# akashsengupta1997/HierarchicalProbabilistic3DHuman

Hardware: AMD Instinct MI355X
Metric: images/sec end-to-end (num_samples=100) (higher is better)
Workload: dtype f32

## Files before the change

hierarchicalprobabilistic3dhuman_amd/_capi.py:

```python
import contextlib
import ctypes
import os

import torch

_PKG_DIR = os.path.dirname(os.path.abspath(__file__))
LIB_PATH = os.path.join(_PKG_DIR, "libhps.so")
DEV_LIB_PATH = os.path.join(_PKG_DIR, "libhps_dev.so")

_c = ctypes
_P = _c.c_void_p
_I = _c.c_int

_PROTOTYPES = {
    "hps_version": [],
    "hps_last_error": [],
    "hps_stream_create_cu_partition": [_I, _I, _c.POINTER(_P)],
    "hps_stream_destroy": [_P],
    "hps_smpl_pose_prep": [_P, _P, _I, _P, _I, _P, _P, _P, _P, _I, _P, _I, _I, _P, _P, _P, _I, _P],
    "hps_smpl_blend": [_P, _P, _P, _P, _I, _I, _I, _I, _I, _I, _P],
    "hps_smpl_lbs": [_P, _I, _P, _P, _P, _I, _I, _P, _P, _I, _I, _P],
    "hps_smpl_mesh_fused": [_P, _P, _P, _P, _P, _P, _I, _I, _P, _P, _I, _I, _I, _I, _I, _P],
    "hps_smpl_mesh_fused_picks": [_P, _P, _P, _P, _P, _P, _I, _I, _P, _P, _I, _I, _I, _I, _I, _P, _P, _I, _P],
    "hps_smpl_mesh_fused_shared_shape": [_P] * 8 + [_I, _I, _P] + [_I] * 5 + [_P, _P, _I, _P],
# ... 6 lines not shown
    "hps_smpl_lbs_backward": [_P, _I, _P, _P, _P, _I, _I, _P, _P, _I, _P, _P, _P, _P, _P, _P, _I, _I, _P],
    "hps_smpl_blend_backward": [_P, _P, _P, _P, _I, _I, _I, _I, _I, _P],
    "hps_smpl_pose_prep_backward": [_P, _P, _I, _P, _I, _P, _P, _P, _P, _I, _P, _P, _I, _P, _I, _P, _P, _P, _I, _P],
    "hps_smpl_joints": [_P, _P, _P, _P, _P, _I, _I, _P, _P, _I, _I, _P],
    "hps_vertex_uncertainty": [_P, _P, _I, _I, _I, _P],
    "hps_joints_and_uncertainty": [_P, _P, _P, _P, _P, _I, _I, _P, _P, _I, _I, _P, _P, _I, _I, _I, _P],
    "hps_query_workspace": [_I, _c.c_int64, _c.c_int64, _c.c_int64],
    "hps_mf_sample": [_P, _P, _P, _P, _P, _I, _I, _I, _I, _c.c_float, _c.c_float, _P, _P, _P, _c.c_uint64,
                      _c.c_int64, _P, _I, _P, _P, _P, _P],
    "hps_infer_assemble": [_P, _P, _P, _P, _P, _P, _P, _I, _I, _I, _I, _P],
    "hps_quat_to_rotmat": [_P, _P, _I, _P],
    "hps_rot6d_to_rotmat": [_P, _P, _I, _P],
    "hps_batch_rodrigues": [_P, _P, _I, _P],
    "hps_linear": [_P, _I, _P, _P, _P, _P, _I, _I, _I, _I, _I, _P],
    "hps_head_trunk": [_P] + [_I] + [_P] * 14 + [_I] * 7 + [_P],
    "hps_head_joint_level": [_P, _I, _I, _P, _I, _P, _P, _P, _P, _P, _P, _P, _P, _P, _c.c_float, _P, _P, _I, _I, _P],
    "hps_head_joint_level_svd": [_P, _I, _I, _P, _I, _P, _P, _P, _P, _P, _P, _P, _P, _P, _c.c_float, _P, _P, _P, _P, _I, _I, _I, _P],
    "hps_svd3_packed": [_P, _P, _I, _I, _P],
    "hps_host_svd3_emulated": [_P, _P, _I, _I],
    "hps_host_svd_flavor": [],
    "hps_host_svd3_packed": [_P, _P, _I, _I],
    "hps_host_bind_lapack": [_c.c_char_p],
    "hps_head_svd_finish": [_P, _P, _I, _P, _P, _P, _P, _P, _P, _I, _I, _P],
    "hps_canny_edges": [_P, _P, _I, _P, _P, _P, _P, _P, _P, _I, _I, _I, _I, _c.c_float, _I, _P],
    "hps_canny_edge_map": [_P, _P, _I, _P, _c.c_int64, _I, _I, _I, _I, _c.c_float, _I, _P],
    "hps_proxy_rep": [_P, _P, _P, _P, _I, _I, _I, _I, _c.c_float, _P],
    "hps_pointset_errors": [_P, _P, _I, _I, _I, _I, _P, _P, _P, _P, _P],
    "hps_heatmaps_to_joints2d": [_P, _P, _P, _I, _I, _I, _c.c_float, _P],
    "hps_sample_joints2d_error": [_P, _P, _I, _P, _P, _P, _c.c_float, _P, _I, _I, _P],
    "hps_conv2d_bn_act_pad": [_P, _P, _P, _P, _P, _P, _I, _I, _I, _I, _I, _I, _I, _I, _I, _I, _I, _I, _I, _I, _I, _P, _P],
    "hps_conv2d_bn_act_pad_down": [_P] * 9 + [_I] * 14 + [_P, _P],
    "hps_conv3x3_winograd": [_P, _P, _P, _P, _P, _P, _I, _I, _I, _I, _I, _I, _I, _I, _P, _P],
    "hps_conv3x3_winograd_workspace": [_I, _I, _I, _I, _I],
    "hps_stem_phase_frames_bytes": [_I, _I, _I],
    "hps_stem_phase_split": [_P, _P, _I, _I, _I, _I, _P],
    "hps_proxy_rep_phase_frames": [_P, _P, _P, _P, _I, _I, _I, _I, _c.c_float, _P],
    "hps_stem_winograd": [_P, _P, _P, _P, _P, _I, _I, _I, _I, _I, _P],
    "hps_stem_pool_side_bytes": [_I, _I, _I],
    "hps_stem_winograd_pooled": [_P, _P, _P, _P, _P, _P, _I, _I, _I, _I, _I, _P],
    "hps_stem_winograd_pooled_nchw": [_P, _P, _P, _P, _P, _P, _I, _I, _I, _I, _I, _P],
    "hps_sums_f64": [_P, _P, _P, _I, _c.c_double, _P, _P, _P, _P],
    "hps_sizeof_enc_op": [],
    "hps_encoder_run": [_P, _I, _P],
    "hps_head_pose_levels": [_P, _I, _I, _P, _P, _I, _P, _P, _P, _P, _P, _P, _P, _P, _P, _c.c_float, _P, _P, _P, _P, _P, _P,
                             _P, _P, _I, _I, _I, _I, _P],
    "hps_nchw_to_padded_nhwc": [_P, _P, _I, _I, _I, _I, _I, _P],
    "hps_nchw_to_padded_nhwc_generic": [_P, _P, _I, _I, _I, _I, _I, _I, _I, _P],
    "hps_maxpool3x3s2_pad": [_P, _P, _I, _I, _I, _I, _I, _P],
    "hps_global_avgpool_pad": [_P, _P, _I, _I, _I, _I, _I, _P],
    "hps_mf_log_norm_const": [_P, _I, _P, _P, _P, _P],
    "hps_mf_nll": [_P, _P, _P, _P, _P, _I, _c.c_double, _P, _P, _P, _P, _P],
    "hps_mf_loss_forward": [_P, _P, _P, _P],
    "hps_mf_loss_backward": [_P, _P, _P, _P],
    "hps_head_forward_refine": [_P, _I] + [_P] * 9 + [_I] + [_P] * 6 + [_c.c_float] + [_P] * 13 + [_I] * 7 + [_P],
    "hps_head_pose_levels_backward": [_P, _I, _I, _P, _P, _I] + [_P] * 21 + [_I, _I, _I, _P],
    "hps_head_pose_levels_backward_factors": [_P, _I, _I, _P, _P, _I] + [_P] * 23 + [_I, _I, _I, _P],
    "hps_mf_sample_keep_quat": [_P, _P, _P, _I, _I, _I, _I, _c.c_float, _c.c_float, _P, _P, _P, _c.c_uint64, _c.c_int64, _I, _P, _P, _P, _P],
    "hps_mf_sample_backward": [_P, _P, _P, _P, _P, _P, _P, _P, _I, _I, _I, _c.c_float, _P, _P, _P, _P],
    "hps_head_trunk_backward": [_P, _I] + [_P] * 20 + [_I] * 7 + [_P],
    "hps_rot6d_to_rotmat_backward": [_P, _P, _P, _I, _P],
    "hps_conv_wgrad": [_P] * 4 + [_I] * 12 + [_P],
    "hps_conv_wgrad_slice_pixels": [_I, _I],
    "hps_conv_wgrad_workspace": [_I] * 9,
    "hps_conv_dgrad": [_P] * 4 + [_I] * 12 + [_P],
    "hps_relu_gate_pad": [_P] * 4 + [_I] * 6 + [_P],
    "hps_relu_gate_workspace": [_I] * 4,
# ... 235 lines not shown
```

hierarchicalprobabilistic3dhuman_amd/csrc/composite.hip:

```cpp
#include <vector>

#include "hps_common.h"

using namespace hps;

extern "C" int hps_sizeof_enc_op(void) { return (int)sizeof(hps_enc_op); }

extern "C" int hps_encoder_run(const hps_enc_op* ops, int n_ops, hps_stream_t stream) {
    if (!ops && n_ops > 0) return bad_arg("hps_encoder_run: null op list");
    for (int i = 0; i < n_ops; ++i) {
        const hps_enc_op& o = ops[i];
        int rc;
        switch (o.kind) {
            case HPS_ENC_RELAYOUT:
                rc = hps_nchw_to_padded_nhwc(o.x, o.y, o.B, o.Cin, o.H, o.W, o.opad, stream);
                break;
            case HPS_ENC_RELAYOUT_GENERIC:
                rc = hps_nchw_to_padded_nhwc_generic(o.x, o.y, o.B, o.Cin, o.Cout, o.H, o.W, o.KW, o.opad, stream);
                break;
            case HPS_ENC_CONV:
                rc = hps_conv2d_bn_act_pad(o.x, o.w, o.scale, o.shift, o.residual, o.y, o.B, o.H, o.W, o.ipad, o.Cin, o.Cout,
                                           o.KH, o.KW, o.stride, o.pad, o.opad, o.relu, o.row_mode, o.variant, o.ksplit,
                                           o.splitk_ws, stream);
                break;
            case HPS_ENC_CONV_DOWN:
                rc = hps_conv2d_bn_act_pad_down(o.x, o.w, o.scale, o.shift, o.y, o.w_down, o.scale_down, o.shift_down, o.y_down, o.B, o.H,
                                                o.W, o.ipad, o.Cin, o.Cout, o.KH, o.KW, o.stride, o.pad, o.opad, o.relu, o.variant, o.ksplit,
                                                o.splitk_ws, stream);
                break;
            case HPS_ENC_CONV_WINOGRAD:
                rc = hps_conv3x3_winograd(o.x, o.w, o.scale, o.shift, o.residual, o.y, o.B, o.H, o.W, o.ipad, o.Cin, o.Cout, o.opad,
                                          o.relu, o.splitk_ws, stream);
                break;
            case HPS_ENC_STEM_SPLIT:
                rc = hps_stem_phase_split(o.x, o.y, o.B, o.Cin, o.H, o.W, stream);
                break;
            case HPS_ENC_STEM_WINOGRAD:
                rc = hps_stem_winograd(o.x, o.w, o.scale, o.shift, o.y, o.B, o.H, o.W, o.opad, o.relu, stream);
                break;
            case HPS_ENC_STEM_WINOGRAD_POOLED:
                rc = hps_stem_winograd_pooled(o.x, o.w, o.scale, o.shift, o.y, o.splitk_ws, o.B, o.H, o.W, o.opad, o.relu, stream);
                break;
            case HPS_ENC_STEM_WINOGRAD_POOLED_NCHW:
                rc = hps_stem_winograd_pooled_nchw(o.x, o.w, o.scale, o.shift, o.y, o.splitk_ws, o.B, o.H, o.W, o.opad, o.relu, stream);
                break;
            case HPS_ENC_MAXPOOL:
                rc = hps_maxpool3x3s2_pad(o.x, o.y, o.B, o.H, o.W, o.Cin, o.opad, stream);
                break;
            case HPS_ENC_AVGPOOL:
                rc = hps_global_avgpool_pad(o.x, o.y, o.B, o.H, o.W, o.Cin, o.ipad, stream);
                break;
            default:
                return bad_arg("hps_encoder_run: unknown op kind");
        }
        if (rc != HPS_OK) return rc;
    }
    return HPS_OK;
}

extern "C" int hps_head_pose_levels(const float* embed, int embed_dim, int hidden, const int32_t* level_joints,
                                    const int32_t* level_sizes_host, int n_levels, const int32_t* anc_ptr,
                                    const int32_t* anc_idx, const float* const* w1t_ptrs, const float* const* b1_ptrs,
                                    const float* const* w2_ptrs, const float* const* b2_ptrs, float* u_proper,
// ... 54 lines not shown
```

hierarchicalprobabilistic3dhuman_amd/csrc/conv_wino.hip:

```cpp
#include <type_traits>

#include "hps_common.h"

namespace hps {

typedef float f32x16 __attribute__((ext_vector_type(16)));

constexpr int WT = 64;
constexpr int WC = 64;
constexpr int WK = 8;
constexpr int W_OPER = 16 * 2 * 64 * 4;
constexpr int W_WIN = 18 * 18;
constexpr int W_RAW = W_WIN * WK;
constexpr int W_RAW_PIECES = (W_WIN * 2 + 63) / 64;

struct WinoGeom {
    int in_row, in_img;
    int out_row, out_img;
    int ipad, opad;
    int blocks_x, blocks_img;
    int Cin, Cout, n_ct, relu;
    int items;
    unsigned magic_ct, magic_img, magic_x;
    int B, ksplit, cps, raw;
    unsigned magic_ks;
};

#ifdef HPS_DEV_BUILD
__device__ unsigned long long g_wino_stamps[256 * 16];
#define WINO_STAMP(k) do { if (ab == 11 && tid == 0 && nth_item == 1) g_wino_stamps[blockIdx.x * 16 + (k)] = clock64(); } while (0)
#else
#define WINO_STAMP(k) do { } while (0)
#endif

__device__ __forceinline__ unsigned wino_div(unsigned n, unsigned d, unsigned magic) {
    unsigned q = __umulhi(n, magic);
    if (n - q * d >= d) ++q;
    return q;
}

template <int AB, bool QUAD, bool W8 = false, bool TR = false>
__global__ __launch_bounds__(W8 ? 512 : 256, 1) void conv_wino_kernel(const float* __restrict__ x, const float* __restrict__ u,
                                                           const float* __restrict__ scale, const float* __restrict__ shift,
                                                           const float* __restrict__ residual, float* __restrict__ y,
                                                           const WinoGeom g) {
    typedef __attribute__((address_space(3))) void* lptr_t;
    extern __shared__ __attribute__((aligned(16))) float smem[];
    float* sA = smem;
    float* sB = smem + 2 * W_OPER;
    float* sR = smem + 4 * W_OPER;
    constexpr int ab = AB;

    constexpr int NW = W8 ? 8 : 4;
    const int tid = threadIdx.x, lane = tid & 63, wave = __builtin_amdgcn_readfirstlane(tid >> 6);
    const int kl = lane >> 5, il = lane & 31;
    const int pg = W8 ? wave >> 2 : 0;
    const int wm = (wave & 3) >> 1, wn = wave & 1;
    const int nchunks = QUAD ? g.cps : g.Cin / WK;
    constexpr int RP = QUAD ? (W8 ? 1 : 2) : (W8 ? 2 : 3);

    unsigned r_off[3];
    int r_img[3];
    bool r_ok[3];
#pragma unroll
    for (int t = 0; t < 3; ++t) {
        const int e = 64 * (wave + NW * t) + lane;
        if (QUAD) {
            const int px = e >> 1;
            r_ok[t] = t < RP;
            r_img[t] = (px >> 6) & 3;
            r_off[t] = (unsigned)((((px >> 3) & 7) * g.in_row + (px & 7) * g.Cin + (e & 1) * 4) * 4);
        } else {
            r_ok[t] = t < RP && (wave + NW * t) < W_RAW_PIECES && e < 2 * W_WIN;
            const int px = r_ok[t] ? (e >> 1) : 0;
// ... 353 lines not shown
#pragma unroll
                for (int e = 0; e < 4; ++e) {
                    const int r = 4 * q + e;
                    const float2 o = xch[(((1 - pg) * 16 + r) * 4 + w4) * 64 + lane];
                    float yv[2];
                    if (pg == 0) {
                        yv[0] = k0[0][r] + k0[1][r] + o.x;
                        yv[1] = k1[0][r] + k1[1][r] + o.y;
                    } else {
                        yv[0] = o.x - k0[0][r] - k0[1][r];
                        yv[1] = o.y - k1[0][r] - k1[1][r];
                    }
                    const float sc = e == 0 ? sc4[q].x : e == 1 ? sc4[q].y : e == 2 ? sc4[q].z : sc4[q].w;
                    const float sh = e == 0 ? sh4[q].x : e == 1 ? sh4[q].y : e == 2 ? sh4[q].z : sh4[q].w;
#pragma unroll
                    for (int a = 0; a < 2; ++a) {
                        float v = yv[a];
                        if (finish) {
                            v = v * sc + sh;
                            if (residual) v += e == 0 ? res[a][q].x : e == 1 ? res[a][q].y : e == 2 ? res[a][q].z : res[a][q].w;
                            if (g.relu) v = fmaxf(v, 0.0f);
                        }
                        out[a][e] = v;
                    }
                }
                if (store_ok) {
#pragma unroll
                    for (int a = 0; a < 2; ++a)
                        *reinterpret_cast<float4*>(y + lane_base + (size_t)a * g.out_row + 8 * q) = make_float4(out[a][0], out[a][1], out[a][2], out[a][3]);
                }
            }
        } else if (W8) {
            const int co = cur_ct * WC + wn * 32 + il;
            const float sc = scale[co], sh = shift[co];
            const size_t lane_base = (QUAD ? cur_out + (size_t)(2 * wm + kl) * g.out_img + co
                                           : cur_out + (size_t)(8 * wm) * g.out_row + (size_t)(8 * kl) * g.Cout + co) + (size_t)pg * g.Cout;
            const bool store_ok = !QUAD || 2 * wm + kl < cur_nimg;
            float2* xch = reinterpret_cast<float2*>(sA);
            float k0[2][16], k1[2][16];
#pragma unroll
            for (int r = 0; r < 16; ++r)
#pragma unroll
                for (int jj = 0; jj < 2; ++jj) {
                    k0[jj][r] = acc[0 + jj][r] + acc[2 + jj][r] + acc[4 + jj][r];
                    k1[jj][r] = acc[2 + jj][r] - acc[4 + jj][r] - acc[6 + jj][r];
                }
            const int w4 = wave & 3;
#pragma unroll
            for (int r = 0; r < 16; ++r) {
                const float2 e = pg == 0 ? make_float2(k0[1][r], k1[1][r]) : make_float2(k0[0][r], k1[0][r]);
                xch[((pg * 16 + r) * 4 + w4) * 64 + lane] = e;
            }
            float res[16][2];
            if (residual) {
#pragma unroll
                for (int r = 0; r < 16; ++r)
#pragma unroll
                    for (int a = 0; a < 2; ++a)
                        res[r][a] = residual[lane_base + (size_t)(2 * (r >> 2) + a) * g.out_row + (size_t)(2 * (r & 3)) * g.Cout];
            }
            WINO_STAMP(3);
            __syncthreads();
            WINO_STAMP(4);
#pragma unroll
            for (int r = 0; r < 16; ++r) {
                const float2 o = xch[(((1 - pg) * 16 + r) * 4 + w4) * 64 + lane];
                float yv[2];
                if (pg == 0) {
                    yv[0] = k0[0][r] + k0[1][r] + o.x;
                    yv[1] = k1[0][r] + k1[1][r] + o.y;
                } else {
                    yv[0] = o.x - k0[0][r] - k0[1][r];
                    yv[1] = o.y - k1[0][r] - k1[1][r];
                }
#pragma unroll
                for (int a = 0; a < 2; ++a) {
                    float v = yv[a];
                    if (!QUAD || !g.raw) {
                        v = v * sc + sh;
                        if (residual) v += res[r][a];
                        if (g.relu) v = fmaxf(v, 0.0f);
                    }
                    if (store_ok) y[lane_base + (size_t)(2 * (r >> 2) + a) * g.out_row + (size_t)(2 * (r & 3)) * g.Cout] = v;
                }
            }
            WINO_STAMP(5);
        } else if (ab != 4) {
            const int co = cur_ct * WC + wn * 32 + il;
            const float sc = scale[co], sh = shift[co];
            const size_t lane_base = QUAD ? cur_out + (size_t)(2 * wm + kl) * g.out_img + co
                                          : cur_out + (size_t)(8 * wm) * g.out_row + (size_t)(8 * kl) * g.Cout + co;
            const bool store_ok = !QUAD || 2 * wm + kl < cur_nimg;
            float res[2][4] = {{0.f, 0.f, 0.f, 0.f}, {0.f, 0.f, 0.f, 0.f}};
            auto load_res = [&](int r, float (&dst)[4]) {
#pragma unroll
                for (int q = 0; q < 4; ++q)
                    dst[q] = residual[lane_base + (size_t)(2 * (r >> 2) + (q >> 1)) * g.out_row + (size_t)(2 * (r & 3) + (q & 1)) * g.Cout];
            };
            if (residual) load_res(0, res[0]);
#pragma unroll
            for (int r = 0; r < 16; ++r) {
                if (residual && r < 15) load_res(r + 1, res[(r + 1) & 1]);
                float s0[4], s1[4];
#pragma unroll
                for (int j = 0; j < 4; ++j) {
                    constexpr int S = W8 ? 0 : 4;
                    s0[j] = acc[0 * S + j][r] + acc[1 * S + j][r] + acc[2 * S + j][r];
                    s1[j] = acc[1 * S + j][r] - acc[2 * S + j][r] - acc[3 * S + j][r];
                }
                float yv[4];
                yv[0] = s0[0] + s0[1] + s0[2];
                yv[1] = s0[1] - s0[2] - s0[3];
                yv[2] = s1[0] + s1[1] + s1[2];
                yv[3] = s1[1] - s1[2] - s1[3];
#pragma unroll
                for (int q = 0; q < 4; ++q) {
// ... 12 lines not shown
            for (int p = 0; p < NP; ++p)
#pragma unroll
                for (int r = 0; r < 16; ++r) t += acc[p][r];
            if (t == 12345.678f) y[0] = t;
        }
        if (next >= g.items) break;
        item = next;
    }
}

__global__ __launch_bounds__(256) void wino_splitk_epilogue_kernel(const float* __restrict__ partial, const float* __restrict__ scale,
                                                                   const float* __restrict__ shift, const float* __restrict__ residual,
                                                                   float* __restrict__ y, int total4, int ksplit, int Cout, int opad,
                                                                   int relu) {
    const int i = blockIdx.x * 256 + threadIdx.x;
    if (i >= total4) return;
    float4 acc = reinterpret_cast<const float4*>(partial)[i];
    for (int k = 1; k < ksplit; ++k) {
        const float4 v = reinterpret_cast<const float4*>(partial)[(size_t)k * total4 + i];
        acc.x += v.x; acc.y += v.y; acc.z += v.z; acc.w += v.w;
    }
    const unsigned e = (unsigned)i * 4u;
    const unsigned m = e / (unsigned)Cout, co = e - m * Cout;
    const unsigned b = m >> 6, py = (m >> 3) & 7, px = m & 7, fw = 8 + 2 * opad;
    const size_t o = ((size_t)(b * fw + py + opad) * fw + px + opad) * Cout + co;
    const float4 sc = *reinterpret_cast<const float4*>(scale + co), sh = *reinterpret_cast<const float4*>(shift + co);
    float4 v = make_float4(acc.x * sc.x + sh.x, acc.y * sc.y + sh.y, acc.z * sc.z + sh.z, acc.w * sc.w + sh.w);
    if (residual) {
        const float4 r = *reinterpret_cast<const float4*>(residual + o);
        v.x += r.x; v.y += r.y; v.z += r.z; v.w += r.w;
    }
    if (relu) { v.x = fmaxf(v.x, 0.f); v.y = fmaxf(v.y, 0.f); v.z = fmaxf(v.z, 0.f); v.w = fmaxf(v.w, 0.f); }
    *reinterpret_cast<float4*>(y + o) = v;
}

#ifdef HPS_DEV_BUILD
constexpr int H_A = 16 * 32 * 4;
constexpr int H_B = 16 * 64 * 4;
constexpr int H_WIN = 10 * 18;
constexpr int H_RAW = 6 * 256;

template <int AB>
__global__ __launch_bounds__(256, 2) void conv_wino_half_kernel(const float* __restrict__ x, const float* __restrict__ u4,
                                                                const float* __restrict__ scale, const float* __restrict__ shift,
                                                                const float* __restrict__ residual, float* __restrict__ y, const WinoGeom g) {
    typedef __attribute__((address_space(3))) void* lptr_t;
    extern __shared__ __attribute__((aligned(16))) float smem[];
    float* sB0 = smem;
    float* sA = smem + H_B;
    float* sB1 = smem + H_B + 2 * H_A;
    float* sR = smem + 2 * H_B + 2 * H_A;
    constexpr int ab = AB;

    const int tid = threadIdx.x, lane = tid & 63, wave = __builtin_amdgcn_readfirstlane(tid >> 6);
    const int kl = lane >> 5, il = lane & 31;
    const int pg = wave >> 1, wn = wave & 1;
    const int nh = g.Cin / 4, n8 = g.Cin / 8;

    unsigned r_off[2];
    bool r_ok[2];
#pragma unroll
    for (int t = 0; t < 2; ++t) {
        const int e = 64 * (wave + 4 * t) + lane;
        r_ok[t] = (t == 0 || wave < 2) && e < 2 * H_WIN;
        const int px = r_ok[t] ? (e >> 1) : 0;
        r_off[t] = (unsigned)(((px / 18) * g.in_row + (px % 18) * g.Cin + (e & 1) * 4) * 4);
// ... 180 lines not shown
                    y[lane_base + (size_t)(2 * (r >> 2) + a) * g.out_row + (size_t)(2 * (r & 3)) * g.Cout] = v;
                }
            }
        }
        if (next >= g.items) break;
        item = next;
    }
}
#endif

static unsigned wino_magic(unsigned d) { return d <= 1 ? 0xffffffffu : (unsigned)(0x100000000ull / d); }

}

using namespace hps;

#ifdef HPS_DEV_BUILD
static int g_wino_quad_ks = 0;
#else
constexpr int g_wino_quad_ks = 0;
#endif
static int wino_quad_ksplit(int Cin) {
    if (g_wino_quad_ks > 0 && (Cin / WK) % g_wino_quad_ks == 0) return g_wino_quad_ks;
    return (Cin / WK) % 4 == 0 && (Cin / WK) / 4 >= 8 ? 4 : 1;
}

extern "C" size_t hps_conv3x3_winograd_workspace(int B, int H, int W, int Cin, int Cout) {
    if (H != 8 || W != 8 || B <= 0 || Cin <= 0 || Cout <= 0) return 0;
    return (size_t)wino_quad_ksplit(Cin) * B * 64 * Cout * sizeof(float);
}

static int wino_launch(const float* x, const float* u, const float* scale, const float* shift, const float* residual,
                       float* y, int B, int H, int W, int ipad, int Cin, int Cout, int opad, int relu, float* splitk_ws, int ablate,
                       hps_stream_t stream) {
    if (!x || !u || !scale || !shift || !y) return bad_arg("hps_conv3x3_winograd: null pointer");
    if (B <= 0) return HPS_OK;
    const bool quad = H == 8 && W == 8;
    if (!quad && (H <= 0 || W <= 0 || (H % 16) || (W % 16)))
        return bad_arg("hps_conv3x3_winograd: H and W must be multiples of 16 (8 x 8 blocks of 2 x 2 tiles), or H = W = 8");
    if (Cin <= 0 || Cin % WK != 0 || Cout <= 0 || Cout % WC != 0) return bad_arg("hps_conv3x3_winograd: Cin % 8 == 0 and Cout % 64 == 0 required");
    if (ipad < 1 || opad < 0) return bad_arg("hps_conv3x3_winograd: the input frame needs a halo of at least one pixel");
    if ((size_t)B * (H + 2 * ipad) * (W + 2 * ipad) * Cin * 4 >= 0xffffffffull || (size_t)B * (H + 2 * opad) * (W + 2 * opad) * Cout * 4 >= 0xffffffffull)
        return bad_arg("hps_conv3x3_winograd: tensor exceeds the 32-bit lane offsets");
    if (quad && !splitk_ws) return bad_arg("hps_conv3x3_winograd: 8 x 8 maps need splitk_ws (hps_conv3x3_winograd_workspace bytes)");
    WinoGeom g;
    g.in_row = (W + 2 * ipad) * Cin;
    g.in_img = (H + 2 * ipad) * g.in_row;
    g.out_row = (W + 2 * opad) * Cout;
    g.out_img = (H + 2 * opad) * g.out_row;
    g.ipad = ipad; g.opad = opad;
    g.blocks_x = W / 16;
    g.blocks_img = (H / 16) * (W / 16);
    g.Cin = Cin; g.Cout = Cout; g.n_ct = Cout / WC; g.relu = relu;
    g.items = B * g.blocks_img * g.n_ct;
    g.B = B; g.ksplit = 1; g.cps = Cin / WK; g.raw = 0;
    if (quad) {
        g.ksplit = wino_quad_ksplit(Cin);
        g.cps = Cin / WK / g.ksplit;
        g.raw = 1;
        g.out_row = 8 * Cout; g.out_img = 64 * Cout; g.opad = 0;
        g.items = ((B + 3) / 4) * g.n_ct * g.ksplit;
    }
    g.magic_ct = wino_magic((unsigned)g.n_ct);
    g.magic_img = wino_magic((unsigned)g.blocks_img);
    g.magic_x = wino_magic((unsigned)g.blocks_x);
    g.magic_ks = wino_magic((unsigned)g.ksplit);
    const size_t lds = (size_t)(4 * W_OPER + 3 * W_RAW) * sizeof(float);
    const dim3 grid((unsigned)(g.items < 256 ? g.items : 256));
    int grant_rc = HPS_OK;
    auto launch = [&](auto AB, auto Q) {
        constexpr int ab = decltype(AB)::value;
        constexpr bool q = decltype(Q)::value;
        if ((grant_rc = grant_lds<&conv_wino_kernel<ab, q>>(160 * 1024, "hps_conv3x3_winograd")) != HPS_OK) return;
        hipLaunchKernelGGL((conv_wino_kernel<ab, q>), grid, dim3(256), lds, (hipStream_t)stream, x, u, scale, shift, quad ? nullptr : residual,
                           quad ? splitk_ws : y, g);
    };
    auto launch8 = [&](auto Q, auto TRF, auto AB) {
        constexpr bool q = decltype(Q)::value, tr = decltype(TRF)::value;
        constexpr int ab = decltype(AB)::value;
        if ((grant_rc = grant_lds<&conv_wino_kernel<ab, q, true, tr>>(160 * 1024, "hps_conv3x3_winograd")) != HPS_OK) return;
        hipLaunchKernelGGL((conv_wino_kernel<ab, q, true, tr>), grid, dim3(512), lds, (hipStream_t)stream, x, u, scale, shift, quad ? nullptr : residual,
                           quad ? splitk_ws : y, g);
    };
    typedef std::integral_constant<int, 0> Z;
    typedef std::integral_constant<bool, false> F;
    typedef std::integral_constant<bool, true> T;
    if (quad) {
        if (ablate != 0 && ablate != 21 && ablate != 23) return bad_arg("hps_conv3x3_winograd: ablations exist for the 16 x 16-block geometry only");
#ifdef HPS_DEV_BUILD
        if (ablate == 21) launch(std::integral_constant<int, 0>(), T());
        else if (ablate == 23) launch8(T(), T(), Z());
        else
#endif
            launch8(T(), F(), Z());
        if (grant_rc != HPS_OK) return grant_rc;
        const int rc = check_launch("hps_conv3x3_winograd");
        if (rc != HPS_OK) return rc;
        const int total4 = B * 64 * Cout / 4;
        hipLaunchKernelGGL(wino_splitk_epilogue_kernel, dim3((unsigned)((total4 + 255) / 256)), dim3(256), 0, (hipStream_t)stream, splitk_ws,
                           scale, shift, residual, y, total4, g.ksplit, Cout, opad, relu);
        return check_launch("hps_conv3x3_winograd (slices)");
    }
    switch (ablate) {
        case 0: launch8(F(), F(), Z()); break;
#ifdef HPS_DEV_BUILD
        case 23: launch8(F(), T(), Z()); break;
        case 24: launch8(F(), F(), std::integral_constant<int, 4>()); break;
        case 31: launch8(F(), F(), std::integral_constant<int, 1>()); break;
        case 33: launch8(F(), F(), std::integral_constant<int, 3>()); break;
        case 35: launch8(F(), F(), std::integral_constant<int, 5>()); break;
        case 36: launch8(F(), F(), std::integral_constant<int, 6>()); break;
        case 40: launch8(F(), F(), std::integral_constant<int, 10>()); break;
        case 42: launch8(F(), F(), std::integral_constant<int, 12>()); break;
        case 43: launch8(F(), F(), std::integral_constant<int, 13>()); break;
        case 44: launch8(F(), F(), std::integral_constant<int, 14>()); break;
        case 11: launch8(F(), F(), std::integral_constant<int, 11>()); break;
        case 21: launch(std::integral_constant<int, 0>(), F()); break;
        case 1: launch(std::integral_constant<int, 1>(), F()); break;
        case 2: launch(std::integral_constant<int, 2>(), F()); break;
        case 3: launch(std::integral_constant<int, 3>(), F()); break;
        case 4: launch(std::integral_constant<int, 4>(), F()); break;
        case 5: launch(std::integral_constant<int, 5>(), F()); break;
        case 6: launch(std::integral_constant<int, 6>(), F()); break;
        case 7: launch(std::integral_constant<int, 7>(), F()); break;
        case 8: launch(std::integral_constant<int, 8>(), F()); break;
        case 9: launch(std::integral_constant<int, 9>(), F()); break;
        case 10: launch(std::integral_constant<int, 10>(), F()); break;
#endif
        default: return bad_arg("hps_conv3x3_winograd: ablate");
    }
    if (grant_rc != HPS_OK) return grant_rc;
    return check_launch("hps_conv3x3_winograd");
}

extern "C" int hps_conv3x3_winograd(const float* x, const float* u, const float* scale, const float* shift, const float* residual,
                                    float* y, int B, int H, int W, int ipad, int Cin, int Cout, int opad, int relu,
                                    float* splitk_ws, hps_stream_t stream) {
    return wino_launch(x, u, scale, shift, residual, y, B, H, W, ipad, Cin, Cout, opad, relu, splitk_ws, 0, stream);
}

#ifdef HPS_DEV_BUILD
extern "C" int hps_dev_conv3x3_winograd_half(const float* x, const float* u4, const float* scale, const float* shift, const float* residual,
                                             float* y, int B, int H, int W, int ipad, int Cin, int Cout, int opad, int relu, int ablate,
                                             int wgs_per_cu, hps_stream_t stream) {
    if (!x || !u4 || !scale || !shift || !y) return bad_arg("hps_dev_conv3x3_winograd_half: null pointer");
    if (B <= 0) return HPS_OK;
    if (H <= 0 || W <= 0 || (H % 16) || (W % 16) || Cin % 8 != 0 || Cout % WC != 0 || ipad < 1 || opad < 0)
        return bad_arg("hps_dev_conv3x3_winograd_half: shape");
    WinoGeom g;
    g.in_row = (W + 2 * ipad) * Cin;
    g.in_img = (H + 2 * ipad) * g.in_row;
    g.out_row = (W + 2 * opad) * Cout;
    g.out_img = (H + 2 * opad) * g.out_row;
    g.ipad = ipad; g.opad = opad;
    g.blocks_x = W / 16;
    g.blocks_img = (H / 16) * (W / 16);
    g.Cin = Cin; g.Cout = Cout; g.n_ct = Cout / WC; g.relu = relu;
    g.items = B * g.blocks_img * 2 * g.n_ct;
    g.B = B; g.ksplit = 1; g.cps = Cin / WK; g.raw = 0;
    g.magic_ct = wino_magic((unsigned)g.n_ct);
    g.magic_img = wino_magic((unsigned)g.blocks_img);
    g.magic_x = wino_magic((unsigned)g.blocks_x);
    g.magic_ks = wino_magic(1u);
    const size_t lds = (size_t)(2 * H_A + 2 * H_B + 3 * H_RAW) * sizeof(float);
    const int wgs = 256 * (wgs_per_cu > 0 ? wgs_per_cu : 2);
    const dim3 grid((unsigned)(g.items < wgs ? g.items : wgs));
    int rc = HPS_OK;
    if (ablate == 4) {
        if ((rc = grant_lds<&conv_wino_half_kernel<4>>(160 * 1024, "hps_dev_conv3x3_winograd_half")) != HPS_OK) return rc;
        hipLaunchKernelGGL((conv_wino_half_kernel<4>), grid, dim3(256), lds, (hipStream_t)stream, x, u4, scale, shift, residual, y, g);
    } else {
// ... 22 lines not shown
```

include/hps.h:

```cpp
#ifndef HPS_H_
#define HPS_H_

#include <stddef.h>
#include <stdint.h>

#ifdef __cplusplus
extern "C" {
#endif
#pragma GCC visibility push(default)

typedef void* hps_stream_t;


#define HPS_OK 0
#define HPS_E_BADARG (-1)
#define HPS_E_UNSUPPORTED (-2)

#define HPS_SVD_HOST 0
#define HPS_SVD_DEVICE 1
#define HPS_SVD_DEVICE_FMA 2

#define HPS_SVD_ROUNDING_REFERENCE 0
#define HPS_SVD_ROUNDING_FMA 1
#define HPS_HEAD_WIDE_WORKGROUPS 0x100
// ... 124 lines not shown
                             float* s_proper, float* mode, float delta_i_weight, float* pose_f, float* pose_u,
                             float* pose_s, float* pose_v, int B, int num_body_joints, int svd_flavor,
                             hps_stream_t stream);

int hps_svd3_packed(const float* f, float* usv, int n, int svd_flavor, hps_stream_t stream);

int hps_host_svd3_emulated(const float* f_host, float* usv_host, int n, int svd_flavor);

int hps_host_svd_flavor(void);

int hps_host_svd3_packed(const float* f_host, float* usv_host, int n, int num_threads);
int hps_host_bind_lapack(const char* library_path);

int hps_head_svd_finish(const float* usv_level, const int32_t* joint_ids, int n_level,
                        float* pose_u, float* pose_s, float* pose_v, float* u_proper,
                        float* s_proper, float* mode, int B, int num_body_joints,
                        hps_stream_t stream);


int hps_conv2d_bn_act_pad(const float* x, const float* wn, const float* scale, const float* shift,
                          const float* residual, float* y, int B, int H, int W, int ipad, int Cin, int Cout,
                          int KH, int KW, int stride, int pad, int opad, int relu, int row_mode, int variant,
                          int ksplit, float* splitk_ws, hps_stream_t stream);

int hps_conv2d_bn_act_pad_down(const float* x, const float* wn, const float* scale, const float* shift, float* y,
                               const float* wn_down, const float* scale_down, const float* shift_down, float* y_down,
                               int B, int H, int W, int ipad, int Cin, int Cout, int KH, int KW, int stride, int pad,
                               int opad, int relu, int variant, int ksplit, float* splitk_ws, hps_stream_t stream);

int hps_conv3x3_winograd(const float* x, const float* u, const float* scale, const float* shift,
                         const float* residual, float* y, int B, int H, int W, int ipad, int Cin, int Cout,
                         int opad, int relu, float* splitk_ws, hps_stream_t stream);
size_t hps_conv3x3_winograd_workspace(int B, int H, int W, int Cin, int Cout);

size_t hps_stem_phase_frames_bytes(int B, int H, int W);
int hps_stem_phase_split(const float* x, float* frames, int B, int C, int H, int W, hps_stream_t stream);
int hps_proxy_rep_phase_frames(const float* edge, const float* joints2d, const float* visib, float* frames, int B, int K, int H,
                               int W, float std, hps_stream_t stream);
int hps_stem_winograd(const float* frames, const float* u, const float* scale, const float* shift, float* y, int B, int H,
                      int W, int opad, int relu, hps_stream_t stream);
size_t hps_stem_pool_side_bytes(int B, int H, int W);
int hps_stem_winograd_pooled(const float* frames, const float* u, const float* scale, const float* shift, float* pooled, float* side,
                             int B, int H, int W, int opad, int relu, hps_stream_t stream);
int hps_stem_winograd_pooled_nchw(const float* x, const float* u, const float* scale, const float* shift, float* pooled, float* side,
                                  int B, int H, int W, int opad, int relu, hps_stream_t stream);

enum { HPS_ENC_RELAYOUT = 0, HPS_ENC_CONV = 1, HPS_ENC_MAXPOOL = 2, HPS_ENC_AVGPOOL = 3, HPS_ENC_CONV_WINOGRAD = 4,
       HPS_ENC_STEM_SPLIT = 5, HPS_ENC_STEM_WINOGRAD = 6,
       HPS_ENC_RELAYOUT_GENERIC = 7 ,
       HPS_ENC_STEM_WINOGRAD_POOLED = 8, HPS_ENC_STEM_WINOGRAD_POOLED_NCHW = 9,
       HPS_ENC_CONV_DOWN = 10  };
typedef struct hps_enc_op {
    int kind;
    const float* x;
    const float* w;
    const float* scale;
    const float* shift;
    const float* residual;
    float* y;
    float* splitk_ws;
    int B, H, W, ipad, Cin, Cout, KH, KW, stride, pad, opad, relu, row_mode, variant, ksplit;
    const float* w_down;
    const float* scale_down;
    const float* shift_down;
    float* y_down;
} hps_enc_op;
// ... 193 lines not shown
```

Before: 22500.

## Fuse global avgpool into 8x8 winograd split-k epilogue and vectorize W8 row stores

When an 8x8 winograd conv is followed directly by a global average pool, the encoder now calls a new entry point. It reduces the split-k slices, applies scale, shift, residual and ReLU, and computes the pooled mean in one epilogue kernel, which removes a separate pool launch and the re-read of the feature map. Separately, the non-quad W8 kernel path now stages results through LDS so that each lane writes float4 rows with float4 scale, shift and residual loads, in place of scalar strided stores. This adds LDS traffic and another template instantiation.

```diff
diff --git a/hierarchicalprobabilistic3dhuman_amd/_capi.py b/hierarchicalprobabilistic3dhuman_amd/_capi.py
--- a/hierarchicalprobabilistic3dhuman_amd/_capi.py
+++ b/hierarchicalprobabilistic3dhuman_amd/_capi.py
@@ -62,6 +62,7 @@
     "hps_conv2d_bn_act_pad_down": [_P] * 9 + [_I] * 14 + [_P, _P],
     "hps_conv3x3_winograd": [_P, _P, _P, _P, _P, _P, _I, _I, _I, _I, _I, _I, _I, _I, _P, _P],
     "hps_conv3x3_winograd_workspace": [_I, _I, _I, _I, _I],
+    "hps_conv3x3_winograd_pooled": [_P] * 7 + [_I] * 8 + [_P, _P],
     "hps_stem_phase_frames_bytes": [_I, _I, _I],
     "hps_stem_phase_split": [_P, _P, _I, _I, _I, _I, _P],
     "hps_proxy_rep_phase_frames": [_P, _P, _P, _P, _I, _I, _I, _I, _c.c_float, _P],
diff --git a/hierarchicalprobabilistic3dhuman_amd/csrc/composite.hip b/hierarchicalprobabilistic3dhuman_amd/csrc/composite.hip
--- a/hierarchicalprobabilistic3dhuman_amd/csrc/composite.hip
+++ b/hierarchicalprobabilistic3dhuman_amd/csrc/composite.hip
@@ -29,6 +29,15 @@
                                                 o.splitk_ws, stream);
                 break;
             case HPS_ENC_CONV_WINOGRAD:
+                if (i + 1 < n_ops && o.H == 8 && o.W == 8) {
+                    const hps_enc_op& p = ops[i + 1];
+                    if (p.kind == HPS_ENC_AVGPOOL && p.x == o.y && p.y && p.B == o.B && p.H == 8 && p.W == 8 && p.Cin == o.Cout && p.ipad == o.opad) {
+                        rc = hps_conv3x3_winograd_pooled(o.x, o.w, o.scale, o.shift, o.residual, o.y, p.y, o.B, o.H, o.W, o.ipad, o.Cin, o.Cout,
+                                                         o.opad, o.relu, o.splitk_ws, stream);
+                        ++i;
+                        break;
+                    }
+                }
                 rc = hps_conv3x3_winograd(o.x, o.w, o.scale, o.shift, o.residual, o.y, o.B, o.H, o.W, o.ipad, o.Cin, o.Cout, o.opad,
                                           o.relu, o.splitk_ws, stream);
                 break;
diff --git a/hierarchicalprobabilistic3dhuman_amd/csrc/conv_wino.hip b/hierarchicalprobabilistic3dhuman_amd/csrc/conv_wino.hip
--- a/hierarchicalprobabilistic3dhuman_amd/csrc/conv_wino.hip
+++ b/hierarchicalprobabilistic3dhuman_amd/csrc/conv_wino.hip
@@ -39,7 +39,7 @@
     return q;
 }
 
-template <int AB, bool QUAD, bool W8 = false, bool TR = false>
+template <int AB, bool QUAD, bool W8 = false, bool TR = false, bool ROWS = (W8 && !TR)>
 __global__ __launch_bounds__(W8 ? 512 : 256, 1) void conv_wino_kernel(const float* __restrict__ x, const float* __restrict__ u,
                                                            const float* __restrict__ scale, const float* __restrict__ shift,
                                                            const float* __restrict__ residual, float* __restrict__ y,
@@ -459,10 +459,22 @@
             }
         } else if (W8) {
             const int co = cur_ct * WC + wn * 32 + il;
-            const float sc = scale[co], sh = shift[co];
+            float sc = 1.0f, sh = 0.0f;
+            if (!ROWS) { sc = scale[co]; sh = shift[co]; }
             const size_t lane_base = (QUAD ? cur_out + (size_t)(2 * wm + kl) * g.out_img + co
                                            : cur_out + (size_t)(8 * wm) * g.out_row + (size_t)(8 * kl) * g.Cout + co) + (size_t)pg * g.Cout;
             const bool store_ok = !QUAD || 2 * wm + kl < cur_nimg;
+            const int tq = lane >> 3, rr = tq >> 1, kk = tq & 1;
+            const int cq = cur_ct * WC + wn * 32 + 4 * (lane & 7);
+            const bool finish = !QUAD || !g.raw;
+            const size_t row_base = QUAD ? cur_out + (size_t)(2 * wm + kk) * g.out_img + (size_t)(2 * rr + pg) * g.Cout + cq
+                                         : cur_out + (size_t)(8 * wm) * g.out_row + (size_t)(2 * (4 * kk + rr) + pg) * g.Cout + cq;
+            const bool row_ok = !QUAD || 2 * wm + kk < cur_nimg;
+            float4 sc4 = make_float4(1.f, 1.f, 1.f, 1.f), sh4 = make_float4(0.f, 0.f, 0.f, 0.f);
+            if (ROWS && finish) {
+                sc4 = *reinterpret_cast<const float4*>(scale + cq);
+                sh4 = *reinterpret_cast<const float4*>(shift + cq);
+            }
             float2* xch = reinterpret_cast<float2*>(sA);
             float k0[2][16], k1[2][16];
 #pragma unroll
@@ -478,37 +490,102 @@
                 const float2 e = pg == 0 ? make_float2(k0[1][r], k1[1][r]) : make_float2(k0[0][r], k1[0][r]);
                 xch[((pg * 16 + r) * 4 + w4) * 64 + lane] = e;
             }
-            float res[16][2];
-            if (residual) {
-#pragma unroll
-                for (int r = 0; r < 16; ++r)
-#pragma unroll
-                    for (int a = 0; a < 2; ++a)
-                        res[r][a] = residual[lane_base + (size_t)(2 * (r >> 2) + a) * g.out_row + (size_t)(2 * (r & 3)) * g.Cout];
-            }
-            WINO_STAMP(3);
-            __syncthreads();
-            WINO_STAMP(4);
-#pragma unroll
-            for (int r = 0; r < 16; ++r) {
-                const float2 o = xch[(((1 - pg) * 16 + r) * 4 + w4) * 64 + lane];
-                float yv[2];
-                if (pg == 0) {
-                    yv[0] = k0[0][r] + k0[1][r] + o.x;
-                    yv[1] = k1[0][r] + k1[1][r] + o.y;
-                } else {
-                    yv[0] = o.x - k0[0][r] - k0[1][r];
-                    yv[1] = o.y - k1[0][r] - k1[1][r];
-                }
-#pragma unroll
-                for (int a = 0; a < 2; ++a) {
-                    float v = yv[a];
-                    if (!QUAD || !g.raw) {
-                        v = v * sc + sh;
-                        if (residual) v += res[r][a];
-                        if (g.relu) v = fmaxf(v, 0.0f);
+            if (ROWS) {
+                float4 res4[8];
+                if (finish && residual && row_ok) {
+#pragma unroll
+                    for (int i = 0; i < 8; ++i) res4[i] = *reinterpret_cast<const float4*>(residual + row_base + (size_t)i * g.out_row);
+                }
+                WINO_STAMP(3);
+                __syncthreads();
+                WINO_STAMP(4);
+                float* stg = sA + ((1 - pg) * 64 + w4) * 128;
+                float2 o[2][4];
+#pragma unroll
+                for (int e = 0; e < 4; ++e) o[0][e] = xch[(((1 - pg) * 16 + e) * 4 + w4) * 64 + lane];
+#pragma unroll
+                for (int q = 0; q < 4; ++q) {
+                    if (q < 3) {
+#pragma unroll
+                        for (int e = 0; e < 4; ++e) o[(q + 1) & 1][e] = xch[(((1 - pg) * 16 + 4 * (q + 1) + e) * 4 + w4) * 64 + lane];
                     }
-                    if (store_ok) y[lane_base + (size_t)(2 * (r >> 2) + a) * g.out_row + (size_t)(2 * (r & 3)) * g.Cout] = v;
+#pragma unroll
+                    for (int e = 0; e < 4; ++e) {
+                        const int r = 4 * q + e;
+                        const float2 ov = o[q & 1][e];
+                        float yv[2];
+                        if (pg == 0) {
+                            yv[0] = k0[0][r] + k0[1][r] + ov.x;
+                            yv[1] = k1[0][r] + k1[1][r] + ov.y;
+                        } else {
+                            yv[0] = ov.x - k0[0][r] - k0[1][r];
+                            yv[1] = ov.y - k1[0][r] - k1[1][r];
+                        }
+                        stg[r * 512 + lane] = yv[0];
+                        stg[r * 512 + 64 + lane] = yv[1];
+                    }
+                }
+                __builtin_amdgcn_fence(__ATOMIC_RELEASE, "wavefront");
+                asm volatile("s_waitcnt lgkmcnt(0)" ::: "memory");
+                __builtin_amdgcn_fence(__ATOMIC_ACQUIRE, "wavefront");
+                const float* rd = stg + rr * 512 + kk * 32 + 4 * (lane & 7);
+                auto write_rows = [&](auto HAS_RES, auto RELU) {
+                    float4 v[8];
+#pragma unroll
+                    for (int i = 0; i < 8; ++i)
+                        v[i] = *reinterpret_cast<const float4*>(rd + (i >> 1) * 2048 + (i & 1) * 64);
+#pragma unroll
+                    for (int i = 0; i < 8; ++i) {
+                        if (finish) {
+                            v[i].x = v[i].x * sc4.x + sh4.x; v[i].y = v[i].y * sc4.y + sh4.y;
+                            v[i].z = v[i].z * sc4.z + sh4.z; v[i].w = v[i].w * sc4.w + sh4.w;
+                            if (decltype(HAS_RES)::value) { v[i].x += res4[i].x; v[i].y += res4[i].y; v[i].z += res4[i].z; v[i].w += res4[i].w; }
+                            if (decltype(RELU)::value) {
+                                v[i].x = fmaxf(v[i].x, 0.0f); v[i].y = fmaxf(v[i].y, 0.0f); v[i].z = fmaxf(v[i].z, 0.0f); v[i].w = fmaxf(v[i].w, 0.0f);
+                            }
+                        }
+                        if (row_ok) *reinterpret_cast<float4*>(y + row_base + (size_t)i * g.out_row) = v[i];
+                    }
+                };
+                typedef std::integral_constant<bool, false> No;
+                typedef std::integral_constant<bool, true> Yes;
+                if (!finish) write_rows(No(), No());
+                else if (residual) { if (g.relu) write_rows(Yes(), Yes()); else write_rows(Yes(), No()); }
+                else if (g.relu) write_rows(No(), Yes());
+                else write_rows(No(), No());
+            } else {
+                float res[16][2];
+                if (residual) {
+#pragma unroll
+                    for (int r = 0; r < 16; ++r)
+#pragma unroll
+                        for (int a = 0; a < 2; ++a)
+                            res[r][a] = residual[lane_base + (size_t)(2 * (r >> 2) + a) * g.out_row + (size_t)(2 * (r & 3)) * g.Cout];
+                }
+                WINO_STAMP(3);
+                __syncthreads();
+                WINO_STAMP(4);
+#pragma unroll
+                for (int r = 0; r < 16; ++r) {
+                    const float2 o = xch[(((1 - pg) * 16 + r) * 4 + w4) * 64 + lane];
+                    float yv[2];
+                    if (pg == 0) {
+                        yv[0] = k0[0][r] + k0[1][r] + o.x;
+                        yv[1] = k1[0][r] + k1[1][r] + o.y;
+                    } else {
+                        yv[0] = o.x - k0[0][r] - k0[1][r];
+                        yv[1] = o.y - k1[0][r] - k1[1][r];
+                    }
+#pragma unroll
+                    for (int a = 0; a < 2; ++a) {
+                        float v = yv[a];
+                        if (!QUAD || !g.raw) {
+                            v = v * sc + sh;
+                            if (residual) v += res[r][a];
+                            if (g.relu) v = fmaxf(v, 0.0f);
+                        }
+                        if (store_ok) y[lane_base + (size_t)(2 * (r >> 2) + a) * g.out_row + (size_t)(2 * (r & 3)) * g.Cout] = v;
+                    }
                 }
             }
             WINO_STAMP(5);
@@ -587,6 +664,41 @@
     }
     if (relu) { v.x = fmaxf(v.x, 0.f); v.y = fmaxf(v.y, 0.f); v.z = fmaxf(v.z, 0.f); v.w = fmaxf(v.w, 0.f); }
     *reinterpret_cast<float4*>(y + o) = v;
+}
+
+__global__ __launch_bounds__(512) void wino_splitk_pool_epilogue_kernel(const float* __restrict__ partial, const float* __restrict__ scale,
+                                                                        const float* __restrict__ shift, const float* __restrict__ residual,
+                                                                        float* __restrict__ y, float* __restrict__ pooled, int total4,
+                                                                        int ksplit, int Cout, int opad, int relu) {
+    __shared__ __attribute__((aligned(16))) float sv[64 * 32];
+    const unsigned groups = (unsigned)Cout / 32u;
+    const unsigned b = blockIdx.x / groups, cg = blockIdx.x - b * groups;
+    const unsigned pix = threadIdx.x >> 3, co = cg * 32u + 4u * (threadIdx.x & 7u);
+    const unsigned m = b * 64u + pix;
+    const size_t i = ((size_t)m * Cout + co) >> 2;
+    float4 acc = reinterpret_cast<const float4*>(partial)[i];
+    for (int k = 1; k < ksplit; ++k) {
+        const float4 v = reinterpret_cast<const float4*>(partial)[(size_t)k * total4 + i];
+        acc.x += v.x; acc.y += v.y; acc.z += v.z; acc.w += v.w;
+    }
+    const unsigned py = (m >> 3) & 7, px = m & 7, fw = 8 + 2 * opad;
+    const size_t o = ((size_t)(b * fw + py + opad) * fw + px + opad) * Cout + co;
+    const float4 sc = *reinterpret_cast<const float4*>(scale + co), sh = *reinterpret_cast<const float4*>(shift + co);
+    float4 v = make_float4(acc.x * sc.x + sh.x, acc.y * sc.y + sh.y, acc.z * sc.z + sh.z, acc.w * sc.w + sh.w);
+    if (residual) {
+        const float4 r = *reinterpret_cast<const float4*>(residual + o);
+        v.x += r.x; v.y += r.y; v.z += r.z; v.w += r.w;
+    }
+    if (relu) { v.x = fmaxf(v.x, 0.f); v.y = fmaxf(v.y, 0.f); v.z = fmaxf(v.z, 0.f); v.w = fmaxf(v.w, 0.f); }
+    *reinterpret_cast<float4*>(y + o) = v;
+    *reinterpret_cast<float4*>(sv + pix * 32 + 4 * (threadIdx.x & 7u)) = v;
+    __syncthreads();
+    if (threadIdx.x < 32) {
+        float sum = 0.0f;
+#pragma unroll 8
+        for (int p = 0; p < 64; ++p) sum += sv[p * 32 + threadIdx.x];
+        pooled[(size_t)b * Cout + cg * 32u + threadIdx.x] = sum / 64.0f;
+    }
 }
 
 #ifdef HPS_DEV_BUILD
@@ -833,10 +945,11 @@
 
 static int wino_launch(const float* x, const float* u, const float* scale, const float* shift, const float* residual,
                        float* y, int B, int H, int W, int ipad, int Cin, int Cout, int opad, int relu, float* splitk_ws, int ablate,
-                       hps_stream_t stream) {
+                       hps_stream_t stream, float* pooled = nullptr) {
     if (!x || !u || !scale || !shift || !y) return bad_arg("hps_conv3x3_winograd: null pointer");
     if (B <= 0) return HPS_OK;
     const bool quad = H == 8 && W == 8;
+    if (pooled && !quad) return bad_arg("hps_conv3x3_winograd_pooled: the average pool rides in the second pass of the 8 x 8 geometry only");
     if (!quad && (H <= 0 || W <= 0 || (H % 16) || (W % 16)))
         return bad_arg("hps_conv3x3_winograd: H and W must be multiples of 16 (8 x 8 blocks of 2 x 2 tiles), or H = W = 8");
     if (Cin <= 0 || Cin % WK != 0 || Cout <= 0 || Cout % WC != 0) return bad_arg("hps_conv3x3_winograd: Cin % 8 == 0 and Cout % 64 == 0 required");
@@ -876,46 +989,56 @@
         hipLaunchKernelGGL((conv_wino_kernel<ab, q>), grid, dim3(256), lds, (hipStream_t)stream, x, u, scale, shift, quad ? nullptr : residual,
                            quad ? splitk_ws : y, g);
     };
-    auto launch8 = [&](auto Q, auto TRF, auto AB) {
-        constexpr bool q = decltype(Q)::value, tr = decltype(TRF)::value;
+    auto launch8 = [&](auto Q, auto TRF, auto AB, auto ROWSF) {
+        constexpr bool q = decltype(Q)::value, tr = decltype(TRF)::value, rows = decltype(ROWSF)::value;
         constexpr int ab = decltype(AB)::value;
-        if ((grant_rc = grant_lds<&conv_wino_kernel<ab, q, true, tr>>(160 * 1024, "hps_conv3x3_winograd")) != HPS_OK) return;
-        hipLaunchKernelGGL((conv_wino_kernel<ab, q, true, tr>), grid, dim3(512), lds, (hipStream_t)stream, x, u, scale, shift, quad ? nullptr : residual,
-                           quad ? splitk_ws : y, g);
+        if ((grant_rc = grant_lds<&conv_wino_kernel<ab, q, true, tr, rows>>(160 * 1024, "hps_conv3x3_winograd")) != HPS_OK) return;
+        hipLaunchKernelGGL((conv_wino_kernel<ab, q, true, tr, rows>), grid, dim3(512), lds, (hipStream_t)stream, x, u, scale, shift,
+                           quad ? nullptr : residual, quad ? splitk_ws : y, g);
     };
     typedef std::integral_constant<int, 0> Z;
     typedef std::integral_constant<bool, false> F;
     typedef std::integral_constant<bool, true> T;
     if (quad) {
-        if (ablate != 0 && ablate != 21 && ablate != 23) return bad_arg("hps_conv3x3_winograd: ablations exist for the 16 x 16-block geometry only");
+        if (ablate != 0 && ablate != 21 && ablate != 23 && ablate != 25 && ablate != 27)
+            return bad_arg("hps_conv3x3_winograd: ablations exist for the 16 x 16-block geometry only");
 #ifdef HPS_DEV_BUILD
         if (ablate == 21) launch(std::integral_constant<int, 0>(), T());
-        else if (ablate == 23) launch8(T(), T(), Z());
+        else if (ablate == 23) launch8(T(), T(), Z(), F());
+        else if (ablate == 27) launch8(T(), F(), Z(), T());
         else
 #endif
-            launch8(T(), F(), Z());
+            launch8(T(), F(), Z(), F());
         if (grant_rc != HPS_OK) return grant_rc;
         const int rc = check_launch("hps_conv3x3_winograd");
         if (rc != HPS_OK) return rc;
         const int total4 = B * 64 * Cout / 4;
+        if (pooled) {
+            hipLaunchKernelGGL(wino_splitk_pool_epilogue_kernel, dim3((unsigned)(B * (Cout / 32))), dim3(512), 0, (hipStream_t)stream, splitk_ws,
+                               scale, shift, residual, y, pooled, total4, g.ksplit, Cout, opad, relu);
+            return check_launch("hps_conv3x3_winograd_pooled (slices)");
+        }
         hipLaunchKernelGGL(wino_splitk_epilogue_kernel, dim3((unsigned)((total4 + 255) / 256)), dim3(256), 0, (hipStream_t)stream, splitk_ws,
                            scale, shift, residual, y, total4, g.ksplit, Cout, opad, relu);
         return check_launch("hps_conv3x3_winograd (slices)");
     }
     switch (ablate) {
-        case 0: launch8(F(), F(), Z()); break;
+        case 0: launch8(F(), F(), Z(), T()); break;
 #ifdef HPS_DEV_BUILD
-        case 23: launch8(F(), T(), Z()); break;
-        case 24: launch8(F(), F(), std::integral_constant<int, 4>()); break;
-        case 31: launch8(F(), F(), std::integral_constant<int, 1>()); break;
-        case 33: launch8(F(), F(), std::integral_constant<int, 3>()); break;
-        case 35: launch8(F(), F(), std::integral_constant<int, 5>()); break;
-        case 36: launch8(F(), F(), std::integral_constant<int, 6>()); break;
-        case 40: launch8(F(), F(), std::integral_constant<int, 10>()); break;
-        case 42: launch8(F(), F(), std::integral_constant<int, 12>()); break;
-        case 43: launch8(F(), F(), std::integral_constant<int, 13>()); break;
-        case 44: launch8(F(), F(), std::integral_constant<int, 14>()); break;
-        case 11: launch8(F(), F(), std::integral_constant<int, 11>()); break;
+        case 23: launch8(F(), T(), Z(), F()); break;
+        case 27: launch8(F(), F(), Z(), T()); break;
+        case 25: launch8(F(), F(), Z(), F()); break;
+        case 26: launch8(F(), F(), std::integral_constant<int, 11>(), F()); break;
+        case 24: launch8(F(), F(), std::integral_constant<int, 4>(), T()); break;
+        case 31: launch8(F(), F(), std::integral_constant<int, 1>(), T()); break;
+        case 33: launch8(F(), F(), std::integral_constant<int, 3>(), T()); break;
+        case 35: launch8(F(), F(), std::integral_constant<int, 5>(), T()); break;
+        case 36: launch8(F(), F(), std::integral_constant<int, 6>(), T()); break;
+        case 40: launch8(F(), F(), std::integral_constant<int, 10>(), T()); break;
+        case 42: launch8(F(), F(), std::integral_constant<int, 12>(), T()); break;
+        case 43: launch8(F(), F(), std::integral_constant<int, 13>(), T()); break;
+        case 44: launch8(F(), F(), std::integral_constant<int, 14>(), T()); break;
+        case 11: launch8(F(), F(), std::integral_constant<int, 11>(), T()); break;
         case 21: launch(std::integral_constant<int, 0>(), F()); break;
         case 1: launch(std::integral_constant<int, 1>(), F()); break;
         case 2: launch(std::integral_constant<int, 2>(), F()); break;
@@ -938,6 +1061,13 @@
                                     float* y, int B, int H, int W, int ipad, int Cin, int Cout, int opad, int relu,
                                     float* splitk_ws, hps_stream_t stream) {
     return wino_launch(x, u, scale, shift, residual, y, B, H, W, ipad, Cin, Cout, opad, relu, splitk_ws, 0, stream);
+}
+
+extern "C" int hps_conv3x3_winograd_pooled(const float* x, const float* u, const float* scale, const float* shift, const float* residual,
+                                           float* y, float* pooled, int B, int H, int W, int ipad, int Cin, int Cout, int opad, int relu,
+                                           float* splitk_ws, hps_stream_t stream) {
+    if (!pooled) return bad_arg("hps_conv3x3_winograd_pooled: null pointer");
+    return wino_launch(x, u, scale, shift, residual, y, B, H, W, ipad, Cin, Cout, opad, relu, splitk_ws, 0, stream, pooled);
 }
 
 #ifdef HPS_DEV_BUILD
diff --git a/include/hps.h b/include/hps.h
--- a/include/hps.h
+++ b/include/hps.h
@@ -180,6 +180,9 @@
                          const float* residual, float* y, int B, int H, int W, int ipad, int Cin, int Cout,
                          int opad, int relu, float* splitk_ws, hps_stream_t stream);
 size_t hps_conv3x3_winograd_workspace(int B, int H, int W, int Cin, int Cout);
+int hps_conv3x3_winograd_pooled(const float* x, const float* u, const float* scale, const float* shift,
+                                const float* residual, float* y, float* pooled, int B, int H, int W, int ipad, int Cin,
+                                int Cout, int opad, int relu, float* splitk_ws, hps_stream_t stream);
 
 size_t hps_stem_phase_frames_bytes(int B, int H, int W);
 int hps_stem_phase_split(const float* x, float* frames, int B, int C, int H, int W, hps_stream_t stream);
```

After: 22650 (median of 6 runs). About the same (+0.7%).
